# syncdoth/face_mask_inpaint

Measured on AMD Instinct MI355X. Metric: train images/sec at 256x256 bs=8 per GPU (PICNet-ref train step), higher is better.
Workload: dtype f32; 1 GPU; train_reference_fill.py PICNet-ref 256x256 fp32, bs=8 per GPU, synthetic CelebA-HQ-shaped batch + random binary_map (BASELINE configs[1]); global_batch=8, parallelism=dp1

## Files before the change

face_mask_inpaint_amd/_lib.py:

```python
from __future__ import annotations

import ctypes as C
import os

_HERE = os.path.dirname(os.path.abspath(__file__))
LIB_PATH = os.path.join(_HERE, "csrc", "libfmi_hip.so")

c_f = C.c_void_p
i32, i64, f32, vp = C.c_int, C.c_int64, C.c_float, C.c_void_p


class ConvDesc(C.Structure):

    _fields_ = [(n, C.c_int) for n in ("N", "H", "W", "C", "OH", "OW", "K", "x_cstride", "y_cstride", "kh", "kw", "stride", "pad", "pad_mode", "dil")] + [("w3", C.c_void_p), ("x3", C.c_void_p), ("y3", C.c_void_p)]


class WeightEntry(C.Structure):
    _fields_ = [("w", vp), ("u", vp), ("v", vp), ("wf", vp), ("wt", vp), ("sigma", vp), ("rows", i32), ("C", i32), ("taps", i32), ("iters", i32), ("wf3", vp), ("wt3", vp)]


class WeightGradEntry(C.Structure):
    _fields_ = [("w", vp), ("u", vp), ("v", vp), ("sigma", vp), ("dwf", vp), ("dw", vp), ("rows", i32), ("C", i32), ("taps", i32), ("pad_", i32)]


# ... 10 lines not shown
SIGNATURES = {
    "fmi_gemm_f32": [vp, vp, vp, i32, i32, i32, i64, i64, i64, i64, i64, i64, i32, i64, i64, i64, f32, f32, vp, vp],
    "fmi_ssim_valid_f32": [vp, vp, vp, i32, i32, i32, i32, f32, f32, vp, vp, i64, vp],
    "fmi_avgpool2_pad_f32": [vp, vp, i32, i32, i32, i32, i32, vp],
    "fmi_resample_u8": [vp, vp, i32, i32, i32, i32, i32, i32, i32, i32, vp, vp, i32, vp],
    "fmi_gather_u8_i64": [vp, vp, i32, i32, i32, i32, i32, vp, vp, vp],
    "fmi_u8_lut_chw_f32": [vp, vp, vp, i32, i32, i32, i32, vp],
    "fmi_split3_f32": [vp, vp, vp, i64, i32, i32, f32, vp],
    "fmi_split3_colsum_f32": [vp, vp, vp, i64, i32, vp],
    "fmi_merge3_f32": [vp, vp, i64, i32, vp],
    "fmi_conv2d_fwd_f32": [PD, vp, vp, vp, vp, vp, i32, i32, i64, vp],
    "fmi_conv2d_dgrad_f32": [PD, vp, vp, vp, vp, vp, i32, i64, vp],
    "fmi_conv_transpose2d_pair_f32": [PD, vp, vp, i32, vp, vp, vp, vp],
    "fmi_conv2d_dgrad_masked_f32": [PD, vp, vp, vp, f32, vp, vp],
    "fmi_conv2d_dgrad_masked_add_f32": [PD, vp, vp, vp, f32, vp, vp, vp],
    "fmi_conv2d_wgrad_f32": [PD, vp, vp, vp, vp, i32, i64, vp],
    "fmi_conv2d_thin_fwd_f32": [PD, vp, vp, vp, vp, vp, i32, vp],
    "fmi_conv2d_thin_dgrad_f32": [PD, vp, vp, vp, vp],
    "fmi_conv2d_thin_input_dgrad_f32": [PD, vp, vp, vp, vp],
    "fmi_conv2d_thin_lrelu_fwd_f32": [PD, vp, f32, vp, vp, vp, i32, vp],
    "fmi_conv2d_thin_lrelu_dgrad_f32": [PD, vp, vp, vp, f32, vp, vp],
    "fmi_conv2d_thin_lrelu_wgrad_f32": [PD, vp, f32, vp, vp, vp, vp],
    "fmi_conv2d_thin_wgrad_f32": [PD, vp, vp, vp, vp, vp],
    "fmi_conv2d_fwd_bf16": [PD, vp, vp, vp, vp, vp, i64, vp],
    "fmi_conv2d_dgrad_bf16": [PD, vp, vp, vp, vp, vp, i64, vp],
    "fmi_conv2d_wgrad_bf16": [PD, vp, vp, vp, vp],
    "fmi_pack_weight_bf16": [vp, vp, i32, i32, i32, vp],
    "fmi_scale_channels_bf16": [vp, vp, vp, i32, i64, i32, vp],
    "fmi_scale_channels_gs_bf16": [vp, vp, vp, vp, i64, i32, i64, i32, vp],
    "fmi_noise_bias_act_bf16": [vp, vp, vp, vp, vp, i64, i32, f32, f32, vp],
    "fmi_noise_bias_act_bwd_bf16": [vp, vp, vp, vp, vp, vp, vp, i64, i64, i32, f32, f32, vp],
    "fmi_upfirdn2d_nhwc_bf16": [vp, vp, vp] + [i32] * 14 + [vp],
    "fmi_styled_out_bwd_bf16": [vp] * 11 + [i64, vp, i32, i64, i32, f32, f32, vp],
    "fmi_conv2d_fwd_act_bf16": [PD, vp, vp, vp, vp, vp, vp, f32, f32, vp, vp],
    "fmi_blur_act_bf16": [vp, vp, vp] + [i32] * 8 + [vp, vp, vp, vp, f32, f32, i32, vp],
    "fmi_torgb_fwd_bf16": [vp, vp, vp, vp, vp, vp, i32, i64, i32, vp],
    "fmi_torgb_bwd_bf16": [vp, vp, vp, vp, vp, vp, i64, vp, vp, vp, i32, i64, i32, vp],
    "fmi_bias_grad_f32": [vp, i64, i32, i32, vp, vp],
    "fmi_reflect_pad_fold_f32": [vp, vp, i32, i32, i32, i32, i32, vp],
    "fmi_weight_prepare_f32": [vp, i32, vp],
    "fmi_weight_grad_f32": [vp, i32, vp, vp],
    "fmi_softmax_rows_f32": [vp, vp, i64, i32, vp],
    "fmi_softmax_rows_bwd_f32": [vp, vp, vp, i64, i32, vp],
    "fmi_attention_fwd_f32": [vp, vp, vp, vp, vp, vp, i32, i32, i32, i32, i32, vp],
    "fmi_attention_bwd_f32": [vp] * 12 + [i32] * 5 + [vp],
    "fmi_eltwise_f32": [i32, vp, vp, vp, i64, f32, vp],
# ... 56 lines not shown
    "fmi_adam_step_dev_guarded_f32": [vp, i32, f32, f32, f32, f32, f32, vp, vp, vp],
    "fmi_ranger_step_f32": [vp, i32, f32, f32, f32, f32, f32, f32, i32, f32, i32, vp],
    "fmi_upfirdn2d_f32": [vp, vp, vp, i32, i32, i32, i32, i32, i32, i32, i32, i32, i32, i32, i32, i32, vp],
    "fmi_upfirdn2d_bf16": [vp, vp, vp, i32, i32, i32, i32, i32, i32, i32, i32, i32, i32, i32, i32, i32, vp],
    "fmi_fused_bias_act_f32": [vp, vp, vp, vp, i64, i32, i32, i32, i32, f32, f32, vp],
    "fmi_fused_bias_act_bf16": [vp, vp, vp, vp, i64, i32, i32, i32, i32, f32, f32, vp],
    "fmi_scale_channels_f32": [vp, vp, vp, i32, i64, i32, vp],
    "fmi_scale_channels_gs_f32": [vp, vp, vp, vp, i64, i32, i64, i32, vp],
    "fmi_sqsum_last_f32": [vp, vp, i64, i32, vp],
    "fmi_sqsum_last_bwd_f32": [vp, vp, vp, i64, i32, vp],
    "fmi_noise_bias_act_bwd_f32": [vp, vp, vp, vp, vp, i64, i32, f32, f32, vp],
    "fmi_upfirdn2d_nhwc_f32": [vp, vp, vp, i32, i32, i32, i32, i32, i32, i32, i32, i32, i32, i32, i32, i32, i32, vp],
    "fmi_prelu_f32": [vp, vp, vp, i64, i32, vp],
    "fmi_prelu_bwd_f32": [vp, vp, vp, vp, vp, vp, i64, i64, i32, vp],
    "fmi_subsample_f32": [vp, vp, i32, i32, i32, i32, i32, i32, vp],
    "fmi_bias_grad_nchw_f32": [vp, i32, i32, i64, vp, vp],
    "fmi_bias_grad_nchw_bf16": [vp, i32, i32, i64, vp, vp],
    "fmi_noise_bias_act_f32": [vp, vp, vp, vp, vp, i64, i32, f32, f32, vp],
}

STATUS = {0: "ok", 1: "bad argument", 2: "unsupported shape/mode", 3: "kernel launch failed"}


PREDICATES = {"fmi_debug_bf16_tile": [i32], "fmi_set_deterministic": [i32], "fmi_get_deterministic": [], "fmi_conv2d_thin_supported": [PD], "fmi_conv2d_bf16_supported": [PD], "fmi_conv2d_thin_lrelu_supported": [PD]}


class FmiError(RuntimeError):
    pass


class Library:

    def __init__(self, path: str = LIB_PATH, strict: bool = True):
        if not os.path.exists(path):
            raise FmiError(
                f"{path} not found: build the HIP extension first (python -c 'import __graft_entry__ as g; g.build()'). "
                "There is no CPU fallback."
            )
        self.path = path
        self.cdll = C.CDLL(path)
        self.missing = []
        for name, argtypes in SIGNATURES.items():
            try:
                fn = getattr(self.cdll, name)
            except AttributeError:
                self.missing.append(name)
                continue
# ... 35 lines not shown
```

face_mask_inpaint_amd/csrc/thinconv.hip:

```cpp
#include "common.h"
#include <cstdlib>

namespace {

__device__ __forceinline__ int reflect1(int i, int n) {
  if (i < 0) i = -i;
  if (i >= n) i = 2 * n - 2 - i;
  return i;
}

struct ThinArgs {
  const float* x;
  const float* w;
  const float* bias;
  const float* res;
  float* y;
  int N, H, W, C, K, xcs, ycs, pad_mode, act;
  int flip = 0;
  float in_slope = 1.f;
  const float* xin = nullptr;
};
__device__ __forceinline__ float4 lrelu4(float4 v, float s) {
  v.x = v.x > 0.f ? v.x : v.x * s, v.y = v.y > 0.f ? v.y : v.y * s, v.z = v.z > 0.f ? v.z : v.z * s, v.w = v.w > 0.f ? v.w : v.w * s;
  return v;
// ... 247 lines not shown
      }
      for (int m = 4; m < 4 * CQ; m <<= 1)
#pragma unroll
        for (int k = 0; k < K; ++k) acc[k] += __shfl_xor(acc[k], m, 64);
      if (live && q == 0) {
        const int o = x * a.ycs;
#pragma unroll
        for (int k = 0; k < K; ++k) {
          float r = acc[k];
          if (a.bias) r += a.bias[k];
          if (rrow) r += rrow[o + k];
          if (a.act == 1) r = tanhf(r);
          else if (a.act == 2) r = fmaxf(r, 0.f);
          yrow[o + k] = r;
        }
      }
    }
  }
}


constexpr int LT_H = 8, LT_W = 32, LT_PITCH = 36;
template <int K>
__global__ void __launch_bounds__(256) thin_fwd_lds_kernel(ThinArgs a, int tiles_x, int tiles_y) {
  __shared__ __attribute__((aligned(16))) float sx[(LT_H + 2) * (LT_W + 2) * LT_PITCH];
  const int tid = threadIdx.x, lane = tid & 63, wid = tid >> 6;
  const int i = lane & 3, q = (lane >> 2) & 7, g = lane >> 5;
  int b = blockIdx.x;
  const int tx = b % tiles_x;
  b /= tiles_x;
  const int ty = b % tiles_y, n = b / tiles_y;
  const int y0 = ty * LT_H, x0 = tx * LT_W;
  float wr[9][4];
#pragma unroll
  for (int t = 0; t < 9; ++t)
#pragma unroll
    for (int e = 0; e < 4; ++e) wr[t][e] = i < K ? a.w[((int64_t)(a.flip ? 8 - t : t) * a.C + 4 * q + e) * K + i] : 0.f;
  const float* img = a.x + (int64_t)n * a.H * a.W * a.xcs;
  constexpr int NPIX = (LT_H + 2) * (LT_W + 2), NLD = (NPIX + 31) / 32;
  float4 stage[NLD];
#pragma unroll
  for (int j = 0; j < NLD; ++j) {
    const int p = (tid >> 3) + 32 * j;
    const int wy = p / (LT_W + 2), wx = p - wy * (LT_W + 2);
    int iy = y0 + wy - 1, ix = x0 + wx - 1;
    if (a.pad_mode) {
      iy = reflect1(iy, a.H);
      ix = reflect1(ix, a.W);
    }
    const bool ok = p < NPIX && (unsigned)iy < (unsigned)a.H && (unsigned)ix < (unsigned)a.W;
    stage[j] = make_float4(0.f, 0.f, 0.f, 0.f);
    if (ok) stage[j] = *reinterpret_cast<const float4*>(img + ((int64_t)iy * a.W + ix) * a.xcs + 4 * (tid & 7));
  }
  if (a.in_slope != 1.f) {
#pragma unroll
    for (int j = 0; j < NLD; ++j) stage[j] = lrelu4(stage[j], a.in_slope);
  }
#pragma unroll
  for (int j = 0; j < NLD; ++j) {
    const int p = (tid >> 3) + 32 * j;
    if (p < NPIX) *reinterpret_cast<float4*>(sx + p * LT_PITCH + 4 * (tid & 7)) = stage[j];
  }
  __syncthreads();
#pragma unroll 1
  for (int it = 0; it < 8; ++it) {
    const int ly = 2 * wid + (it >> 2), lx = (it & 3) * 8 + g * 4 + i;
    const float* base = sx + (ly * (LT_W + 2) + lx) * LT_PITCH + 4 * q;
    f32x4_t acc = {0.f, 0.f, 0.f, 0.f};
#pragma unroll
    for (int t = 0; t < 9; ++t) {
      const float4 v = *reinterpret_cast<const float4*>(base + ((t / 3) * (LT_W + 2) + (t % 3)) * LT_PITCH);
      acc = __builtin_amdgcn_mfma_f32_4x4x1f32(wr[t][0], v.x, acc, 0, 0, 0);
      acc = __builtin_amdgcn_mfma_f32_4x4x1f32(wr[t][1], v.y, acc, 0, 0, 0);
      acc = __builtin_amdgcn_mfma_f32_4x4x1f32(wr[t][2], v.z, acc, 0, 0, 0);
      acc = __builtin_amdgcn_mfma_f32_4x4x1f32(wr[t][3], v.w, acc, 0, 0, 0);
    }
#pragma unroll
    for (int m = 4; m < 32; m <<= 1)
#pragma unroll
      for (int k = 0; k < K; ++k) acc[k] += __shfl_xor(acc[k], m, 64);
    const int oy = y0 + ly, ox = x0 + lx;
    if (q < K && oy < a.H && ox < a.W) {
      const int64_t o = ((int64_t)(n * a.H + oy) * a.W + ox) * a.ycs + q;
      float r = acc[0];
#pragma unroll
      for (int k = 1; k < K; ++k) r = q == k ? acc[k] : r;
      if (a.bias) r += a.bias[q];
      if (a.res) r += a.res[o];
      if (a.act == 1) r = tanhf(r);
      else if (a.act == 2) r = fmaxf(r, 0.f);
      a.y[o] = r;
    }
  }
}


template <int K>
__global__ void __launch_bounds__(256) thin_wgrad_lds_kernel(ThinArgs a, float* __restrict__ dwf, float* __restrict__ dbias, int tiles_x,
                                                             int tiles_y, int ntiles) {
  __shared__ __attribute__((aligned(16))) float sx[(LT_H + 2) * (LT_W + 2) * LT_PITCH];
  float(*red)[8] = reinterpret_cast<float(*)[8]>(sx);
  const int tid = threadIdx.x, lane = tid & 63, wid = tid >> 6;
  const int j = lane & 7, grp = lane >> 3;
  float acc[9][4][K], bacc[K];
#pragma unroll
  for (int t = 0; t < 9; ++t)
#pragma unroll
    for (int e = 0; e < 4; ++e)
#pragma unroll
      for (int k = 0; k < K; ++k) acc[t][e][k] = 0.f;
#pragma unroll
  for (int k = 0; k < K; ++k) bacc[k] = 0.f;
  constexpr int NPIX = (LT_H + 2) * (LT_W + 2), NLD = (NPIX + 31) / 32;
  for (int tile = blockIdx.x; tile < ntiles; tile += gridDim.x) {
    int b = tile;
// ... 123 lines not shown
        if (!cok) px = 0;
#pragma unroll
        for (int r = 0; r < 3; ++r) {
          struct __attribute__((packed, aligned(4))) GK {
            float e[K];
          };
          const GK g = *reinterpret_cast<const GK*>(gp[r] + px * a.ycs);
#pragma unroll
          for (int k = 0; k < K; ++k) gv[r * 3 + c][k] = (cok && rok[r]) ? g.e[k] : 0.f;
        }
      }
      f32x4_t acc = {0.f, 0.f, 0.f, 0.f};
#pragma unroll
      for (int t = 0; t < 9; ++t)
#pragma unroll
        for (int k = 0; k < K; ++k) acc = __builtin_amdgcn_mfma_f32_4x4x1f32(wr[t][k], gv[t][k], acc, 0, 0, 0);
      if (live) {
        float4 o = make_float4(acc[0], acc[1], acc[2], acc[3]);
        if (a.xin) o = lrelu_mask4(o, *reinterpret_cast<const float4*>(a.xin + (xrow - dx) + (int64_t)x * a.xcs), a.in_slope);
        *reinterpret_cast<float4*>(xrow + (int64_t)x * a.xcs) = o;
      }
    }
  }
}

bool thin_shape_ok(const fmi_conv_desc* d) {
  const int cg = d->C / 4;
  return d->dil <= 1 && (int64_t)d->N * d->H * d->W < (1ll << 31) && d->K >= 1 && d->K <= 4 && d->kh == 3 && d->kw == 3 && d->stride == 1 && d->pad == 1 && d->C % 4 == 0 && cg >= 1 &&
         cg <= 16 && (cg & (cg - 1)) == 0 && d->x_cstride % 4 == 0 && d->H >= 3 && d->W >= 3 && d->OH == d->H && d->OW == d->W;
}

}

#define THIN_DISPATCH(KERNEL, ...)                                                              \
  switch (d->K) {                                                                               \
    case 1: hipLaunchKernelGGL((KERNEL<1>), dim3(grid), dim3(256), 0, st, __VA_ARGS__); break;  \
    case 2: hipLaunchKernelGGL((KERNEL<2>), dim3(grid), dim3(256), 0, st, __VA_ARGS__); break;  \
    case 3: hipLaunchKernelGGL((KERNEL<3>), dim3(grid), dim3(256), 0, st, __VA_ARGS__); break;  \
    default: hipLaunchKernelGGL((KERNEL<4>), dim3(grid), dim3(256), 0, st, __VA_ARGS__); break; \
  }

extern "C" int fmi_conv2d_thin_supported(const fmi_conv_desc* d) { return d && thin_shape_ok(d) ? 1 : 0; }

static bool thin_lrelu_ok(const fmi_conv_desc* d) { return thin_shape_ok(d) && d->C == 32; }
extern "C" int fmi_conv2d_thin_lrelu_supported(const fmi_conv_desc* d) { return d && thin_lrelu_ok(d) ? 1 : 0; }

static int thin_fwd_impl(const fmi_conv_desc* d, const float* x, float in_slope, const float* wf, const float* bias, const float* residual,
                         float* y, int act, void* stream) {
  if (!d || !x || !wf || !y || act < 0 || act > 2) return FMI_ERR_BAD_ARG;
  if (!thin_shape_ok(d) || ((uintptr_t)x & 15)) return FMI_ERR_UNSUPPORTED;
  if (in_slope != 1.f && !thin_lrelu_ok(d)) return FMI_ERR_UNSUPPORTED;
  hipStream_t st = (hipStream_t)stream;
  ThinArgs a{x, wf, bias, residual, y, d->N, d->H, d->W, d->C, d->K, d->x_cstride, d->y_cstride, d->pad_mode, act};
  a.in_slope = in_slope;
  const int G = d->C / 4;
  const int64_t total = (int64_t)d->N * d->H * d->W;
  if (total >= (1ll << 31)) return FMI_ERR_UNSUPPORTED;
  int qbits = 0;
  while ((1 << qbits) < G) ++qbits;
  if (d->C == 32) {
    const int tiles_x = (d->W + LT_W - 1) / LT_W, tiles_y = (d->H + LT_H - 1) / LT_H;
    const int64_t nb = (int64_t)d->N * tiles_x * tiles_y;
    if (nb < (1ll << 31)) {
      const int grid = (int)nb;
      THIN_DISPATCH(thin_fwd_lds_kernel, a, tiles_x, tiles_y);
      return fmi_launch_status();
    }
  }
  const int segs = (d->W + SEG - 1) / SEG, ntasks = d->N * d->H * segs;
  const int grid = ntasks / 4 > 8192 ? 8192 : (ntasks + 3) / 4;
  THIN_DISPATCH(thin_fwd_mfma_kernel, a, qbits, ntasks, segs);
  return fmi_launch_status();
}

extern "C" int fmi_conv2d_thin_fwd_f32(const fmi_conv_desc* d, const float* x, const float* wf, const float* bias,
                                       const float* residual, float* y, int act, void* stream) {
  return thin_fwd_impl(d, x, 1.f, wf, bias, residual, y, act, stream);
}
extern "C" int fmi_conv2d_thin_lrelu_fwd_f32(const fmi_conv_desc* d, const float* x, float in_slope, const float* wf, const float* bias,
                                             float* y, int act, void* stream) {
  return thin_fwd_impl(d, x, in_slope, wf, bias, nullptr, y, act, stream);
}

static int thin_dgrad_impl(const fmi_conv_desc* d, const float* dy, const float* wt, const float* xin, float in_slope, float* dx,
                           void* stream) {
  if (!d || !dy || !wt || !dx) return FMI_ERR_BAD_ARG;
  if (!thin_shape_ok(d) || ((uintptr_t)dx & 15) || ((uintptr_t)xin & 15)) return FMI_ERR_UNSUPPORTED;
  hipStream_t st = (hipStream_t)stream;
// ... 39 lines not shown
  const int grid = ntasks / 4 > 8192 ? 8192 : (ntasks + 3) / 4;
  switch (d->C) {
    case 1: hipLaunchKernelGGL((thin_fwd_mfma_kernel<1>), dim3(grid), dim3(256), 0, st, a, qbits, ntasks, segs); break;
    case 2: hipLaunchKernelGGL((thin_fwd_mfma_kernel<2>), dim3(grid), dim3(256), 0, st, a, qbits, ntasks, segs); break;
    case 3: hipLaunchKernelGGL((thin_fwd_mfma_kernel<3>), dim3(grid), dim3(256), 0, st, a, qbits, ntasks, segs); break;
    default: hipLaunchKernelGGL((thin_fwd_mfma_kernel<4>), dim3(grid), dim3(256), 0, st, a, qbits, ntasks, segs); break;
  }
  return fmi_launch_status();
}

static int thin_wgrad_impl(const fmi_conv_desc* d, const float* x, float in_slope, const float* dy, float* dwf, float* dbias, void* stream) {
  if (!d || !x || !dy || !dwf) return FMI_ERR_BAD_ARG;
  if (!thin_shape_ok(d) || ((uintptr_t)x & 15)) return FMI_ERR_UNSUPPORTED;
  if (in_slope != 1.f && !thin_lrelu_ok(d)) return FMI_ERR_UNSUPPORTED;
  hipStream_t st = (hipStream_t)stream;
  ThinArgs a{x, nullptr, nullptr, nullptr, const_cast<float*>(dy), d->N, d->H, d->W, d->C, d->K, d->x_cstride, d->y_cstride, d->pad_mode, 0};
  a.in_slope = in_slope;
  const int G = d->C / 4;
  const int64_t total = (int64_t)d->N * d->H * d->W;
  if (d->C == 32) {
    const int tiles_x = (d->W + LT_W - 1) / LT_W, tiles_y = (d->H + LT_H - 1) / LT_H;
    const int64_t nt = (int64_t)d->N * tiles_x * tiles_y;
    if (nt < (1ll << 31)) {
      const int grid = fmi_det() ? 1 : (nt < 768 ? (int)nt : 768);
      THIN_DISPATCH(thin_wgrad_lds_kernel, a, dwf, dbias, tiles_x, tiles_y, (int)nt);
      return fmi_launch_status();
    }
  }
  const int64_t waves = (total + 64 / G - 1) / (64 / G);
  const int grid = fmi_det() ? 1 : (int)(waves / 4 > 1024 ? 1024 : (waves + 3) / 4);
  THIN_DISPATCH(thin_wgrad_kernel, a, dwf, dbias, G, total);
  return fmi_launch_status();
}
extern "C" int fmi_conv2d_thin_wgrad_f32(const fmi_conv_desc* d, const float* x, const float* dy, float* dwf, float* dbias,
                                         void* stream) {
  return thin_wgrad_impl(d, x, 1.f, dy, dwf, dbias, stream);
}
extern "C" int fmi_conv2d_thin_lrelu_wgrad_f32(const fmi_conv_desc* d, const float* x, float in_slope, const float* dy, float* dwf,
                                               float* dbias, void* stream) {
  return thin_wgrad_impl(d, x, in_slope, dy, dwf, dbias, stream);
}
```

face_mask_inpaint_amd/functional.py:

```python
from __future__ import annotations

import ctypes as C
import math
from typing import List, Optional, Sequence, Tuple

import torch

from . import _lib
from ._lib import ConvDesc, FmiError

EW_LRELU, EW_LRELU_BWD, EW_TANH_BWD, EW_ADD, EW_SCALE, EW_AXPY, EW_MUL, EW_RELU_BWD_OUT, EW_SOFTPLUS, EW_SOFTPLUS_BWD, EW_SUB, EW_RSQRT, EW_RSQRT_BWD, EW_SIGMOID, EW_SIGMOID_BWD = range(15)
ACT_NONE, ACT_TANH, ACT_RELU = 0, 1, 2

ATTN_CHUNK_BYTES = 96 * 1024 * 1024

PROFILE = None


class _prof:
    def __init__(self, tag, flops):
        self.tag, self.flops = tag, flops

    def __enter__(self):
        if PROFILE is not None:
# ... 369 lines not shown


class _ThinConvLReLU(torch.autograd.Function):

    @staticmethod
    def forward(ctx, x, wf, bias, wt, slope, pad_mode, act):
        _chk(x, wf, bias)
        n, h, w, c = x.shape
        k = wf.shape[2]
        d, oh, ow = conv_desc(n, h, w, c, k, 3, 3, 1, 1, pad_mode)
        y = torch.empty((n, oh, ow, k), device=x.device, dtype=torch.float32)
        with _prof(f"conv_fwd|{n}x{h}x{w} {c}->{k} k3s1", 2.0 * n * oh * ow * k * c * 9):
            _L().conv2d_thin_lrelu_fwd_f32(C.byref(d), _p(x), slope, _p(wf), _p(bias), _p(y), act, _st())
        ctx.save_for_backward(x, wf, y if act else None)
        ctx.wt, ctx.cfg, ctx.has_b = wt, (slope, pad_mode, act), bias is not None
        return y

    @staticmethod
    def backward(ctx, gy):
        lib = _L()
        x, wf, y = ctx.saved_tensors
        slope, pad_mode, act = ctx.cfg
        gy = gy.contiguous()
        if act:
            gy = _act_bwd(gy, y, act)
        n, h, w, c = x.shape
        k = wf.shape[2]
        d, _, _ = conv_desc(n, h, w, c, k, 3, 3, 1, 1, pad_mode)
        gx = gwf = gb = None
        if ctx.needs_input_grad[0]:
            gx = torch.empty_like(x)
            with _prof(f"conv_dgrad|{n}x{h}x{w} {c}->{k} k3s1", 2.0 * gy.numel() * c * 9):
                lib.conv2d_thin_lrelu_dgrad_f32(C.byref(d), _p(gy), _p(ctx.wt), _p(x), slope, _p(gx), _st())
        if ctx.needs_input_grad[1]:
            gwf = _zeros_like(wf)
            if ctx.has_b and ctx.needs_input_grad[2]:
                gb = _zeros(k, x.device, torch.float32)
            with _prof(f"conv_wgrad|{n}x{h}x{w} {c}->{k} k3s1", 2.0 * gy.numel() * c * 9):
                lib.conv2d_thin_lrelu_wgrad_f32(C.byref(d), _p(x), slope, _p(gy), _p(gwf), _p(gb), _st())
        elif ctx.has_b and ctx.needs_input_grad[2]:
            gb = _zeros(k, x.device, torch.float32)
            lib.bias_grad_f32(_p(gy), gy.numel() // k, k, k, _p(gb), _st())
        return gx, gwf, gb, None, None, None, None


def lrelu_conv2d(x, pw: PackedWeight, bias=None, slope=0.1, pad=1, pad_mode=0, act=ACT_NONE):
    if x.dtype == torch.float32 and pw.kh == 3 and pw.kw == 3 and pad == 1 and x.is_cuda:
        n, h, w, c = x.shape
        d, _, _ = conv_desc(n, h, w, c, pw.wf.shape[2], 3, 3, 1, 1, pad_mode)
        if _L().conv2d_thin_lrelu_supported(C.byref(d)) and x.data_ptr() % 16 == 0:
            return _ThinConvLReLU.apply(x, pw.wf, bias, pw.wt, float(slope), pad_mode, act)
    return conv2d(leaky_relu(x, slope), pw, bias, None, 1, pad, pad_mode, act)
# ... 1718 lines not shown
```

include/fmi_hip.h:

```cpp
#ifndef FMI_HIP_H
#define FMI_HIP_H

#include <stdint.h>

#ifdef __cplusplus
extern "C" {
#endif

typedef enum {
  FMI_OK = 0,
  FMI_ERR_BAD_ARG = 1,
  FMI_ERR_UNSUPPORTED = 2,
  FMI_ERR_LAUNCH = 3
} fmi_status;

const char* fmi_status_string(int status);
int fmi_version(void);
int fmi_set_deterministic(int on);
int fmi_get_deterministic(void);

int fmi_debug_bf16_tile(int mode);

int fmi_gemm_f32(const float* A, const float* B, float* C, int M, int N, int K,
                 int64_t sa_m, int64_t sa_k, int64_t sb_k, int64_t sb_n, int64_t sc_m, int64_t sc_n,
// ... 27 lines not shown
                       const float* residual, float* y, int act, int batch_w, int64_t w_bstride, void* stream);
int fmi_conv_transpose2d_pair_f32(const fmi_conv_desc* d, const float* x1, const float* x2, int K2, const void* w3b, const float* bias,
                                  float* y, void* stream);
int fmi_conv2d_dgrad_f32(const fmi_conv_desc* d, const float* dy, const float* wt, const float* bias,
                         const float* residual, float* dx, int batch_w, int64_t w_bstride, void* stream);
int fmi_conv2d_dgrad_masked_f32(const fmi_conv_desc* d, const float* dy, const float* wt, const float* mask, float mask_slope, float* dx,
                                void* stream);
int fmi_conv2d_dgrad_masked_add_f32(const fmi_conv_desc* d, const float* dy, const float* wt, const float* mask, float mask_slope,
                                    const float* gadd, float* dx, void* stream);
int fmi_conv2d_wgrad_f32(const fmi_conv_desc* d, const float* x, const float* dy, float* dwf, float* dbias,
                         int batch_w, int64_t w_bstride, void* stream);
int fmi_conv2d_thin_supported(const fmi_conv_desc* d);
int fmi_conv2d_thin_fwd_f32(const fmi_conv_desc* d, const float* x, const float* wf, const float* bias,
                            const float* residual, float* y, int act, void* stream);
int fmi_conv2d_thin_dgrad_f32(const fmi_conv_desc* d, const float* dy, const float* wt, float* dx, void* stream);
int fmi_conv2d_thin_wgrad_f32(const fmi_conv_desc* d, const float* x, const float* dy, float* dwf, float* dbias, void* stream);
int fmi_conv2d_thin_lrelu_supported(const fmi_conv_desc* d);
int fmi_conv2d_thin_lrelu_fwd_f32(const fmi_conv_desc* d, const float* x, float in_slope, const float* wf, const float* bias, float* y, int act,
                                  void* stream);
int fmi_conv2d_thin_lrelu_dgrad_f32(const fmi_conv_desc* d, const float* dy, const float* wt, const float* x, float in_slope, float* dx,
                                    void* stream);
int fmi_conv2d_thin_lrelu_wgrad_f32(const fmi_conv_desc* d, const float* x, float in_slope, const float* dy, float* dwf, float* dbias,
                                    void* stream);
int fmi_conv2d_thin_input_dgrad_f32(const fmi_conv_desc* d, const float* dy, const float* wt, float* dx, void* stream);
int fmi_conv2d_bf16_supported(const fmi_conv_desc* d);
int fmi_conv2d_fwd_bf16(const fmi_conv_desc* d, const uint16_t* x, const uint16_t* wnk, const float* colscale, uint16_t* y, float* ws,
                        int64_t ws_floats, void* stream);
int fmi_conv2d_fwd_act_bf16(const fmi_conv_desc* d, const uint16_t* x, const uint16_t* wnk, const float* colscale, const float* noise,
                            const float* nw, const float* bias, float slope, float gain, uint16_t* y, void* stream);
int fmi_conv2d_dgrad_bf16(const fmi_conv_desc* d, const uint16_t* dy, const uint16_t* wck, const float* colscale, uint16_t* dx, float* ws,
                          int64_t ws_floats, void* stream);
int fmi_conv2d_wgrad_bf16(const fmi_conv_desc* d, const uint16_t* x, const uint16_t* dy, float* dwf, void* stream);
int fmi_pack_weight_bf16(const float* src_tab, uint16_t* dst_bta, int T, int A, int B, void* stream);
int fmi_scale_channels_bf16(const uint16_t* x, const float* s, uint16_t* y, int N, int64_t P, int C, void* stream);
int fmi_scale_channels_gs_bf16(const uint16_t* g, const uint16_t* x, float* gs, float* ws, int64_t ws_floats, int N, int64_t P, int C,
                               void* stream);
int fmi_noise_bias_act_bf16(const uint16_t* x, const float* bias, const float* noise, const float* nw, uint16_t* y, int64_t pixels, int C,
                            float alpha, float scale, void* stream);
int fmi_noise_bias_act_bwd_bf16(const uint16_t* g, const uint16_t* y, const float* noise, uint16_t* gx, float* gnw, float* gbias,
                                float* ws, int64_t ws_floats, int64_t pixels, int C, float alpha, float scale, void* stream);
int fmi_upfirdn2d_nhwc_bf16(const uint16_t* in, const float* kernel, uint16_t* out, int N, int in_h, int in_w, int C, int kh, int kw,
                            int up_x, int up_y, int down_x, int down_y, int pad_x0, int pad_x1, int pad_y0, int pad_y1, void* stream);
int fmi_blur_act_bf16(const uint16_t* in, const float* kernel, uint16_t* out, int N, int in_h, int in_w, int C, int pad_x0, int pad_x1,
                      int pad_y0, int pad_y1, const float* colscale, const float* noise, const float* nw, const float* bias, float slope,
                      float gain, int separable, void* stream);
int fmi_styled_out_bwd_bf16(const uint16_t* g, const uint16_t* y, const float* noise, const float* colscale, const float* nw,
// ... 206 lines not shown
```

Baseline: 102.3 images/s.

## Fuse thin lrelu conv dgrad, wgrad and tanh backward into one persistent kernel

Adds a fused backward kernel for the thin (few output channel) 3x3 conv with input leaky-relu. In one pass it computes the input gradient, the weight and bias gradients via per-block partial rows and a row-sum reduction, and optionally applies the tanh derivative, with reflect-pad folding handled separately for border tiles. The forward LDS kernel becomes persistent with prefetch of the next tile window, and the wgrad grid is sized from occupancy queries. This aims to cut separate dgrad/wgrad/activation launches and repeated reads of x and dy, at the cost of a workspace allocation and considerable kernel complexity.

```diff
diff --git a/face_mask_inpaint_amd/_lib.py b/face_mask_inpaint_amd/_lib.py
--- a/face_mask_inpaint_amd/_lib.py
+++ b/face_mask_inpaint_amd/_lib.py
@@ -56,6 +56,7 @@
     "fmi_conv2d_thin_lrelu_dgrad_f32": [PD, vp, vp, vp, f32, vp, vp],
     "fmi_conv2d_thin_lrelu_wgrad_f32": [PD, vp, f32, vp, vp, vp, vp],
     "fmi_conv2d_thin_wgrad_f32": [PD, vp, vp, vp, vp, vp],
+    "fmi_conv2d_thin_lrelu_bwd_f32": [PD, vp, f32, vp, vp, vp, vp, vp, vp, vp, i64, vp],
     "fmi_conv2d_fwd_bf16": [PD, vp, vp, vp, vp, vp, i64, vp],
     "fmi_conv2d_dgrad_bf16": [PD, vp, vp, vp, vp, vp, i64, vp],
     "fmi_conv2d_wgrad_bf16": [PD, vp, vp, vp, vp],
@@ -158,7 +159,7 @@
 STATUS = {0: "ok", 1: "bad argument", 2: "unsupported shape/mode", 3: "kernel launch failed"}
 
 
-PREDICATES = {"fmi_debug_bf16_tile": [i32], "fmi_set_deterministic": [i32], "fmi_get_deterministic": [], "fmi_conv2d_thin_supported": [PD], "fmi_conv2d_bf16_supported": [PD], "fmi_conv2d_thin_lrelu_supported": [PD]}
+PREDICATES = {"fmi_debug_bf16_tile": [i32], "fmi_set_deterministic": [i32], "fmi_get_deterministic": [], "fmi_conv2d_thin_supported": [PD], "fmi_conv2d_bf16_supported": [PD], "fmi_conv2d_thin_lrelu_supported": [PD], "fmi_conv2d_thin_lrelu_bwd_ws_bytes": [PD]}
 
 
 class FmiError(RuntimeError):
diff --git a/face_mask_inpaint_amd/csrc/thinconv.hip b/face_mask_inpaint_amd/csrc/thinconv.hip
--- a/face_mask_inpaint_amd/csrc/thinconv.hip
+++ b/face_mask_inpaint_amd/csrc/thinconv.hip
@@ -293,75 +293,98 @@
 
 constexpr int LT_H = 8, LT_W = 32, LT_PITCH = 36;
 template <int K>
-__global__ void __launch_bounds__(256) thin_fwd_lds_kernel(ThinArgs a, int tiles_x, int tiles_y) {
+__global__ void __launch_bounds__(256) thin_fwd_lds_kernel(ThinArgs a, int tiles_x, int tiles_y, int ntiles) {
   __shared__ __attribute__((aligned(16))) float sx[(LT_H + 2) * (LT_W + 2) * LT_PITCH];
   const int tid = threadIdx.x, lane = tid & 63, wid = tid >> 6;
   const int i = lane & 3, q = (lane >> 2) & 7, g = lane >> 5;
-  int b = blockIdx.x;
-  const int tx = b % tiles_x;
-  b /= tiles_x;
-  const int ty = b % tiles_y, n = b / tiles_y;
-  const int y0 = ty * LT_H, x0 = tx * LT_W;
   float wr[9][4];
 #pragma unroll
   for (int t = 0; t < 9; ++t)
 #pragma unroll
     for (int e = 0; e < 4; ++e) wr[t][e] = i < K ? a.w[((int64_t)(a.flip ? 8 - t : t) * a.C + 4 * q + e) * K + i] : 0.f;
-  const float* img = a.x + (int64_t)n * a.H * a.W * a.xcs;
   constexpr int NPIX = (LT_H + 2) * (LT_W + 2), NLD = (NPIX + 31) / 32;
   float4 stage[NLD];
-#pragma unroll
-  for (int j = 0; j < NLD; ++j) {
-    const int p = (tid >> 3) + 32 * j;
-    const int wy = p / (LT_W + 2), wx = p - wy * (LT_W + 2);
-    int iy = y0 + wy - 1, ix = x0 + wx - 1;
-    if (a.pad_mode) {
-      iy = reflect1(iy, a.H);
-      ix = reflect1(ix, a.W);
-    }
-    const bool ok = p < NPIX && (unsigned)iy < (unsigned)a.H && (unsigned)ix < (unsigned)a.W;
-    stage[j] = make_float4(0.f, 0.f, 0.f, 0.f);
-    if (ok) stage[j] = *reinterpret_cast<const float4*>(img + ((int64_t)iy * a.W + ix) * a.xcs + 4 * (tid & 7));
-  }
-  if (a.in_slope != 1.f) {
-#pragma unroll
-    for (int j = 0; j < NLD; ++j) stage[j] = lrelu4(stage[j], a.in_slope);
-  }
-#pragma unroll
-  for (int j = 0; j < NLD; ++j) {
-    const int p = (tid >> 3) + 32 * j;
-    if (p < NPIX) *reinterpret_cast<float4*>(sx + p * LT_PITCH + 4 * (tid & 7)) = stage[j];
-  }
-  __syncthreads();
+  auto load_window = [&](int tile) {
+    const int tx = tile % tiles_x;
+    tile /= tiles_x;
+    const int ty = tile % tiles_y, n = tile / tiles_y;
+    const int y0 = ty * LT_H, x0 = tx * LT_W;
+    const float* img = a.x + (int64_t)n * a.H * a.W * a.xcs;
+#pragma unroll
+    for (int j = 0; j < NLD; ++j) {
+      const int p = (tid >> 3) + 32 * j;
+      const int wy = p / (LT_W + 2), wx = p - wy * (LT_W + 2);
+      int iy = y0 + wy - 1, ix = x0 + wx - 1;
+      if (a.pad_mode) {
+        iy = reflect1(iy, a.H);
+        ix = reflect1(ix, a.W);
+      }
+      const bool ok = p < NPIX && (unsigned)iy < (unsigned)a.H && (unsigned)ix < (unsigned)a.W;
+      stage[j] = make_float4(0.f, 0.f, 0.f, 0.f);
+      if (ok) stage[j] = *reinterpret_cast<const float4*>(img + ((int64_t)iy * a.W + ix) * a.xcs + 4 * (tid & 7));
+    }
+  };
+  int tile = blockIdx.x;
+  load_window(tile);
+  while (true) {
+    if (a.in_slope != 1.f) {
+#pragma unroll
+      for (int j = 0; j < NLD; ++j) stage[j] = lrelu4(stage[j], a.in_slope);
+    }
+#pragma unroll
+    for (int j = 0; j < NLD; ++j) {
+      const int p = (tid >> 3) + 32 * j;
+      if (p < NPIX) *reinterpret_cast<float4*>(sx + p * LT_PITCH + 4 * (tid & 7)) = stage[j];
+    }
+    __syncthreads();
+    int b = tile;
+    const int tx = b % tiles_x;
+    b /= tiles_x;
+    const int ty = b % tiles_y, n = b / tiles_y;
+    const int y0 = ty * LT_H, x0 = tx * LT_W;
+    const int next = tile + gridDim.x;
+    if (next < ntiles) load_window(next);
+    float fin[K];
+#pragma unroll
+    for (int k = 0; k < K; ++k) fin[k] = 0.f;
 #pragma unroll 1
-  for (int it = 0; it < 8; ++it) {
-    const int ly = 2 * wid + (it >> 2), lx = (it & 3) * 8 + g * 4 + i;
-    const float* base = sx + (ly * (LT_W + 2) + lx) * LT_PITCH + 4 * q;
-    f32x4_t acc = {0.f, 0.f, 0.f, 0.f};
-#pragma unroll
-    for (int t = 0; t < 9; ++t) {
-      const float4 v = *reinterpret_cast<const float4*>(base + ((t / 3) * (LT_W + 2) + (t % 3)) * LT_PITCH);
-      acc = __builtin_amdgcn_mfma_f32_4x4x1f32(wr[t][0], v.x, acc, 0, 0, 0);
-      acc = __builtin_amdgcn_mfma_f32_4x4x1f32(wr[t][1], v.y, acc, 0, 0, 0);
-      acc = __builtin_amdgcn_mfma_f32_4x4x1f32(wr[t][2], v.z, acc, 0, 0, 0);
-      acc = __builtin_amdgcn_mfma_f32_4x4x1f32(wr[t][3], v.w, acc, 0, 0, 0);
-    }
-#pragma unroll
-    for (int m = 4; m < 32; m <<= 1)
-#pragma unroll
-      for (int k = 0; k < K; ++k) acc[k] += __shfl_xor(acc[k], m, 64);
-    const int oy = y0 + ly, ox = x0 + lx;
-    if (q < K && oy < a.H && ox < a.W) {
-      const int64_t o = ((int64_t)(n * a.H + oy) * a.W + ox) * a.ycs + q;
-      float r = acc[0];
-#pragma unroll
-      for (int k = 1; k < K; ++k) r = q == k ? acc[k] : r;
-      if (a.bias) r += a.bias[q];
-      if (a.res) r += a.res[o];
-      if (a.act == 1) r = tanhf(r);
-      else if (a.act == 2) r = fmaxf(r, 0.f);
-      a.y[o] = r;
-    }
+    for (int it = 0; it < 8; ++it) {
+      const int ly = 2 * wid + (it >> 2), lx = (it & 3) * 8 + g * 4 + i;
+      const float* base = sx + (ly * (LT_W + 2) + lx) * LT_PITCH + 4 * q;
+      f32x4_t acc = {0.f, 0.f, 0.f, 0.f};
+#pragma unroll
+      for (int t = 0; t < 9; ++t) {
+        const float4 v = *reinterpret_cast<const float4*>(base + ((t / 3) * (LT_W + 2) + (t % 3)) * LT_PITCH);
+        acc = __builtin_amdgcn_mfma_f32_4x4x1f32(wr[t][0], v.x, acc, 0, 0, 0);
+        acc = __builtin_amdgcn_mfma_f32_4x4x1f32(wr[t][1], v.y, acc, 0, 0, 0);
+        acc = __builtin_amdgcn_mfma_f32_4x4x1f32(wr[t][2], v.z, acc, 0, 0, 0);
+        acc = __builtin_amdgcn_mfma_f32_4x4x1f32(wr[t][3], v.w, acc, 0, 0, 0);
+      }
+#pragma unroll
+      for (int m = 4; m < 32; m <<= 1)
+#pragma unroll
+        for (int k = 0; k < K; ++k) acc[k] += __shfl_xor(acc[k], m, 64);
+#pragma unroll
+      for (int k = 0; k < K; ++k) fin[k] = it == q ? acc[k] : fin[k];
+    }
+    {
+      const int oy = y0 + 2 * wid + (q >> 2), ox = x0 + (q & 3) * 8 + g * 4 + i;
+      if (oy < a.H && ox < a.W) {
+        const int64_t o = ((int64_t)(n * a.H + oy) * a.W + ox) * a.ycs;
+#pragma unroll
+        for (int k = 0; k < K; ++k) {
+          float r = fin[k];
+          if (a.bias) r += a.bias[k];
+          if (a.res) r += a.res[o + k];
+          if (a.act == 1) r = tanhf(r);
+          else if (a.act == 2) r = fmaxf(r, 0.f);
+          a.y[o + k] = r;
+        }
+      }
+    }
+    if (next >= ntiles) break;
+    tile = next;
+    __syncthreads();
   }
 }
 
@@ -531,6 +554,339 @@
       }
     }
   }
+}
+
+constexpr int BW_W = LT_W + 2, BW_CELLS = (LT_H + 2) * (LT_W + 2), BW_LD = (BW_CELLS + 255) / 256;
+constexpr int BWD_MAX_ROWS = 2048;
+
+template <int P>
+__device__ __forceinline__ float quad_bcast(float v) {
+  return __builtin_bit_cast(float, __builtin_amdgcn_update_dpp(0, __builtin_bit_cast(int, v), P * 0x55, 0xf, 0xf, true));
+}
+
+struct FoldFlags {
+  bool y0, y2, x0, x2;
+};
+__device__ __forceinline__ FoldFlags fold_flags(int pad_mode, int oy, int ox, int H, int W) {
+  FoldFlags f;
+  f.y0 = pad_mode && oy == 1, f.y2 = pad_mode && oy == H - 2, f.x0 = pad_mode && ox == 1, f.x2 = pad_mode && ox == W - 2;
+  return f;
+}
+__device__ __forceinline__ float4 sel4(bool c, float4 v) { return c ? v : make_float4(0.f, 0.f, 0.f, 0.f); }
+__device__ __forceinline__ float4 add4(float4 a, float4 b) { return make_float4(a.x + b.x, a.y + b.y, a.z + b.z, a.w + b.w); }
+
+template <bool FOLD, int TY, int TX>
+__device__ __forceinline__ float4 bwd_g4(const float4* wp, FoldFlags f) {
+  constexpr int o = (2 - TY) * BW_W + (2 - TX);
+  constexpr int dr = (TY == 0 ? -2 : 2) * BW_W, dc = TX == 0 ? -2 : 2;
+  float4 v = wp[o];
+  if constexpr (FOLD) {
+    const bool ey = TY == 0 ? f.y0 : TY == 2 ? f.y2 : false, ex = TX == 0 ? f.x0 : TX == 2 ? f.x2 : false;
+    if constexpr (TY != 1) v = add4(v, sel4(ey, wp[o + dr]));
+    if constexpr (TX != 1) v = add4(v, sel4(ex, wp[o + dc]));
+    if constexpr (TY != 1 && TX != 1) v = add4(v, sel4(ey && ex, wp[o + dr + dc]));
+  }
+  return v;
+}
+template <bool FOLD, int TY, int TX>
+__device__ __forceinline__ float bwd_g1(const float* w1, FoldFlags f) {
+  constexpr int o = 4 * ((2 - TY) * BW_W + (2 - TX));
+  constexpr int dr = 4 * (TY == 0 ? -2 : 2) * BW_W, dc = 4 * (TX == 0 ? -2 : 2);
+  float v = w1[o];
+  if constexpr (FOLD) {
+    const bool ey = TY == 0 ? f.y0 : TY == 2 ? f.y2 : false, ex = TX == 0 ? f.x0 : TX == 2 ? f.x2 : false;
+    if constexpr (TY != 1) v += ey ? w1[o + dr] : 0.f;
+    if constexpr (TX != 1) v += ex ? w1[o + dc] : 0.f;
+    if constexpr (TY != 1 && TX != 1) v += (ey && ex) ? w1[o + dr + dc] : 0.f;
+  }
+  return v;
+}
+
+struct BwdTile {
+  int n, y0, x0;
+};
+struct BwdTiling {
+  int tiles_x, tiles_y, ix0, ix1, iy0, iy1;
+  __host__ __device__ int iw() const { return ix1 - ix0; }
+  __host__ __device__ int ih() const { return iy1 - iy0; }
+  __host__ __device__ int per_image(bool border) const { return border ? tiles_x * tiles_y - iw() * ih() : iw() * ih(); }
+};
+template <bool BORDER>
+__device__ __forceinline__ BwdTile bwd_tile(int tile, const BwdTiling& g) {
+  BwdTile t;
+  const int per = g.per_image(BORDER);
+  t.n = tile / per;
+  int j = tile - t.n * per, tx, ty;
+  if (!BORDER) {
+    ty = g.iy0 + j / g.iw();
+    tx = g.ix0 + j % g.iw();
+  } else {
+    const int full = (g.tiles_y - g.ih()) * g.tiles_x;
+    if (j < full) {
+      const int r = j / g.tiles_x;
+      tx = j - r * g.tiles_x;
+      ty = r < g.iy0 ? r : r - g.iy0 + g.iy1;
+    } else {
+      j -= full;
+      const int side = g.tiles_x - g.iw(), r = j / side, c = j - r * side;
+      ty = g.iy0 + r;
+      tx = c < g.ix0 ? c : c - g.ix0 + g.ix1;
+    }
+  }
+  t.y0 = ty * LT_H, t.x0 = tx * LT_W;
+  return t;
+}
+
+struct BwdArgs {
+  const float* x;
+  const float* dy;
+  const float* yt;
+  const float* wt;
+  float* dx;
+  float* ws;
+  int N, H, W, xcs, ycs, pad_mode;
+  float slope;
+};
+
+template <int K>
+struct __attribute__((packed, aligned(4))) GKv {
+  float e[K];
+};
+
+template <int K>
+__device__ __forceinline__ void bwd_win_load(const BwdArgs& a, BwdTile t, int tid, GKv<K> (&g)[BW_LD], GKv<K> (&yv)[BW_LD], bool (&inner)[BW_LD]) {
+#pragma unroll
+  for (int l = 0; l < BW_LD; ++l) {
+    const int p = tid + 256 * l;
+    const int wy = p / BW_W, wx = p - wy * BW_W;
+    const int py = t.y0 + wy - 1, px = t.x0 + wx - 1;
+    const bool ok = p < BW_CELLS && (unsigned)py < (unsigned)a.H && (unsigned)px < (unsigned)a.W;
+    inner[l] = ok && wy >= 1 && wy <= LT_H && wx >= 1 && wx <= LT_W;
+#pragma unroll
+    for (int k = 0; k < K; ++k) g[l].e[k] = 0.f, yv[l].e[k] = 0.f;
+    if (ok) {
+      const int64_t o = ((int64_t)(t.n * a.H + py) * a.W + px) * a.ycs;
+      g[l] = *reinterpret_cast<const GKv<K>*>(a.dy + o);
+      if (a.yt) yv[l] = *reinterpret_cast<const GKv<K>*>(a.yt + o);
+    }
+  }
+}
+template <int K>
+__device__ __forceinline__ void bwd_win_store(float4* win, int tid, const GKv<K> (&g)[BW_LD], const GKv<K> (&yv)[BW_LD], const bool (&inner)[BW_LD],
+                                              float (&bacc)[K]) {
+#pragma unroll
+  for (int l = 0; l < BW_LD; ++l) {
+    const int p = tid + 256 * l;
+    float v[4] = {0.f, 0.f, 0.f, 0.f};
+#pragma unroll
+    for (int k = 0; k < K; ++k) {
+      v[k] = g[l].e[k] * (1.f - yv[l].e[k] * yv[l].e[k]);
+      bacc[k] += inner[l] ? v[k] : 0.f;
+    }
+    if (p < BW_CELLS) win[p] = make_float4(v[0], v[1], v[2], v[3]);
+  }
+}
+
+__device__ __forceinline__ int64_t bwd_x_uoff(const BwdArgs& a, BwdTile t, int it) {
+  return ((int64_t)(t.n * a.H + t.y0 + (it >> 2)) * a.W + t.x0 + (it & 3) * 8) * a.xcs;
+}
+struct BwdLane {
+  int xlo;
+  int ry, rx;
+};
+__device__ __forceinline__ float4 bwd_x_load(const BwdArgs& a, BwdTile t, int it, BwdLane l, bool valid) {
+  const bool in = valid && t.y0 + l.ry + (it >> 2) < a.H && t.x0 + l.rx + (it & 3) * 8 < a.W;
+  const float* p = a.x + bwd_x_uoff(a, t, it) + l.xlo;
+  return *reinterpret_cast<const float4*>(in ? p : a.x);
+}
+
+constexpr int BWD_PF = 4;
+template <int K, bool FOLD>
+__device__ __forceinline__ void bwd_tile_compute(const BwdArgs& a, const float4* win, BwdTile t, BwdTile nx, bool hasn, BwdLane l, int g, int i,
+                                                 const float (&wr)[9][K], f32x4_t (&dw)[9], float4 (&xr)[BWD_PF]) {
+  static_assert(BWD_PF == 4, "one pass of the unrolled loop = one tile row of the wave");
+#pragma unroll
+  for (int h = 0; h < 2; ++h) {
+    const float4* wrow = win + (l.ry + h) * BW_W + l.rx;
+    const float* grow = reinterpret_cast<const float*>(win + (l.ry + h) * BW_W + 4 * g) + i;
+    const int oy = t.y0 + l.ry + h;
+#pragma unroll
+    for (int j = 0; j < 4; ++j) {
+      const int it = 4 * h + j;
+      const int ox = t.x0 + l.rx + 8 * j;
+      const bool live = oy < a.H && ox < a.W;
+      const float4 xv = sel4(live, xr[j]);
+      xr[j] = h == 0 ? bwd_x_load(a, t, it + 4, l, true) : bwd_x_load(a, nx, it - 4, l, hasn);
+      {
+        const FoldFlags f = fold_flags(a.pad_mode, oy, ox, a.H, a.W);
+        f32x4_t acc[3];
+#pragma unroll
+        for (int r = 0; r < 3; ++r) acc[r] = f32x4_t{0.f, 0.f, 0.f, 0.f};
+#define BWD_TAP(TY, TX)                                                                                                                  \
+  {                                                                                                                                      \
+    const float4 gq = bwd_g4<FOLD, TY, TX>(wrow + 8 * j, f);                                                                             \
+    const float ge[4] = {gq.x, gq.y, gq.z, gq.w};                                                                                        \
+    _Pragma("unroll") for (int k = 0; k < K; ++k) acc[TY] = __builtin_amdgcn_mfma_f32_4x4x1f32(wr[TY * 3 + TX][k], ge[k], acc[TY], 0, 0, 0); \
+  }
+        BWD_TAP(0, 0) BWD_TAP(1, 0) BWD_TAP(2, 0) BWD_TAP(0, 1) BWD_TAP(1, 1) BWD_TAP(2, 1) BWD_TAP(0, 2) BWD_TAP(1, 2) BWD_TAP(2, 2)
+#undef BWD_TAP
+        if (live) {
+          const float4 o = make_float4(acc[0][0] + acc[1][0] + acc[2][0], acc[0][1] + acc[1][1] + acc[2][1], acc[0][2] + acc[1][2] + acc[2][2],
+                                       acc[0][3] + acc[1][3] + acc[2][3]);
+          *reinterpret_cast<float4*>(a.dx + bwd_x_uoff(a, t, it) + l.xlo) = lrelu_mask4(o, xv, a.slope);
+        }
+      }
+      const float4 lv = lrelu4(xv, a.slope);
+#define BWD_PIX(P)                                                                                                                           \
+  {                                                                                                                                          \
+    const float b0 = quad_bcast<P>(lv.x), b1 = quad_bcast<P>(lv.y), b2 = quad_bcast<P>(lv.z), b3 = quad_bcast<P>(lv.w);                      \
+    const float b = i == 0 ? b0 : i == 1 ? b1 : i == 2 ? b2 : b3;                                             \
+    const FoldFlags f = fold_flags(a.pad_mode, oy, t.x0 + 4 * g + 8 * j + P, a.H, a.W);                                                      \
+    BWD_WTAP(P, 0, 0) BWD_WTAP(P, 0, 1) BWD_WTAP(P, 0, 2) BWD_WTAP(P, 1, 0) BWD_WTAP(P, 1, 1) BWD_WTAP(P, 1, 2) BWD_WTAP(P, 2, 0) BWD_WTAP(P, 2, 1) \
+    BWD_WTAP(P, 2, 2)                                                                                                                        \
+  }
+#define BWD_WTAP(P, TY, TX) dw[TY * 3 + TX] = __builtin_amdgcn_mfma_f32_4x4x1f32(bwd_g1<FOLD, TY, TX>(grow + 4 * (8 * j + P), f), b, dw[TY * 3 + TX], 0, 0, 0);
+      BWD_PIX(0) BWD_PIX(1) BWD_PIX(2) BWD_PIX(3)
+#undef BWD_WTAP
+#undef BWD_PIX
+    }
+  }
+}
+
+template <int K, bool FOLD>
+__global__ void __launch_bounds__(256) __attribute__((amdgpu_waves_per_eu((!FOLD && K <= 3) ? 3 : 2))) thin_lrelu_bwd_kernel(BwdArgs a, BwdTiling tg, int ntiles, int row0) {
+  __shared__ __attribute__((aligned(16))) float4 win[2][BW_CELLS];
+  __shared__ float red[9 * 4 * 32];
+  __shared__ float lds4[4];
+  const int tid = threadIdx.x, lane = tid & 63, wid = tid >> 6;
+  const int i = lane & 3, q = (lane >> 2) & 7, g = lane >> 5;
+  float wr[9][K];
+#pragma unroll
+  for (int t = 0; t < 9; ++t)
+#pragma unroll
+    for (int k = 0; k < K; ++k) wr[t][k] = a.wt[(t * K + k) * 32 + 4 * q + i];
+  f32x4_t dw[9];
+#pragma unroll
+  for (int t = 0; t < 9; ++t) dw[t] = f32x4_t{0.f, 0.f, 0.f, 0.f};
+  float bacc[K];
+#pragma unroll
+  for (int k = 0; k < K; ++k) bacc[k] = 0.f;
+  GKv<K> sg[BW_LD], sy[BW_LD];
+  bool inner[BW_LD];
+  float4 xr[BWD_PF];
+
+  int tile = blockIdx.x;
+  BwdTile cur = bwd_tile<FOLD>(tile, tg);
+  bwd_win_load<K>(a, cur, tid, sg, sy, inner);
+  const BwdLane l{(2 * wid * a.W + 4 * g + i) * a.xcs + 4 * q, 2 * wid, 4 * g + i};
+#pragma unroll
+  for (int it = 0; it < BWD_PF; ++it) xr[it] = bwd_x_load(a, cur, it, l, true);
+  bwd_win_store<K>(win[0], tid, sg, sy, inner, bacc);
+  __syncthreads();
+  int pb = 0;
+  for (; tile < ntiles; tile += gridDim.x) {
+    const bool hasn = tile + (int)gridDim.x < ntiles;
+    const BwdTile nx = bwd_tile<FOLD>(hasn ? tile + gridDim.x : tile, tg);
+    if (hasn) bwd_win_load<K>(a, nx, tid, sg, sy, inner);
+    bwd_tile_compute<K, FOLD>(a, win[pb], cur, nx, hasn, l, g, i, wr, dw, xr);
+    if (hasn) bwd_win_store<K>(win[pb ^ 1], tid, sg, sy, inner, bacc);
+    __syncthreads();
+    pb ^= 1;
+    cur = nx;
+  }
+#pragma unroll
+  for (int t = 0; t < 9; ++t)
+#pragma unroll
+    for (int r = 0; r < 4; ++r) dw[t][r] += __shfl_xor(dw[t][r], 32, 64);
+  for (int w = 0; w < 4; ++w) {
+    if (wid == w && g == 0) {
+#pragma unroll
+      for (int t = 0; t < 9; ++t)
+#pragma unroll
+        for (int r = 0; r < 4; ++r) {
+          float* p = red + (t * 4 + r) * 32 + (lane & 31);
+          *p = w == 0 ? dw[t][r] : *p + dw[t][r];
+        }
+    }
+    __syncthreads();
+  }
+  constexpr int RW = 9 * 32 * K + K;
+  float* row = a.ws + (int64_t)(row0 + blockIdx.x) * RW;
+  for (int idx = tid; idx < 9 * 32 * K; idx += 256) {
+    const int t = idx / (32 * K), rem = idx - t * 32 * K, c = rem / K, k = rem - c * K;
+    row[idx] = red[(t * 4 + k) * 32 + c];
+  }
+#pragma unroll
+  for (int k = 0; k < K; ++k) {
+    const float s_ = block_sum_256(bacc[k], lds4);
+    if (tid == 0) row[9 * 32 * K + k] = s_;
+  }
+}
+
+__global__ void __launch_bounds__(1024) thin_sum_rows_kernel(const float* __restrict__ ws, float* __restrict__ dwf, float* __restrict__ dbias, int rows,
+                                                             int width, int nw) {
+  __shared__ float part[32][33];
+  const int tx = threadIdx.x & 31, ty = threadIdx.x >> 5;
+  const int i = blockIdx.x * 32 + tx;
+  float s4[4] = {0.f, 0.f, 0.f, 0.f};
+  if (i < width) {
+    int r = ty;
+    for (; r + 96 < rows; r += 128) {
+#pragma unroll
+      for (int u = 0; u < 4; ++u) s4[u] += ws[(int64_t)(r + 32 * u) * width + i];
+    }
+    for (int u = 0; r < rows; r += 32, ++u) s4[u] += ws[(int64_t)r * width + i];
+  }
+  part[ty][tx] = (s4[0] + s4[1]) + (s4[2] + s4[3]);
+  __syncthreads();
+  if (ty == 0 && i < width) {
+    float t = 0.f;
+#pragma unroll
+    for (int l = 0; l < 32; ++l) t += part[l][tx];
+    if (i < nw) dwf[i] = t;
+    else if (dbias) dbias[i - nw] = t;
+  }
+}
+
+template <typename F>
+static int resident_grid(F kernel) {
+  int per_cu = 0, dev = 0, cus = 0;
+  if (hipOccupancyMaxActiveBlocksPerMultiprocessor(&per_cu, kernel, 256, 0) != hipSuccess || per_cu < 1) per_cu = 1;
+  if (hipGetDevice(&dev) != hipSuccess || hipDeviceGetAttribute(&cus, hipDeviceAttributeMultiprocessorCount, dev) != hipSuccess || cus < 1) cus = 256;
+  (void)hipGetLastError();
+  return per_cu * cus;
+}
+template <int K, bool FOLD>
+static int bwd_resident_grid() {
+  static const int g = resident_grid(thin_lrelu_bwd_kernel<K, FOLD>);
+  return g;
+}
+template <int K>
+static void bwd_launch(const fmi_conv_desc* d, const BwdArgs& a, int64_t rows, hipStream_t st, int* rows_used) {
+  BwdTiling tg{(d->W + LT_W - 1) / LT_W, (d->H + LT_H - 1) / LT_H, 0, 0, 0, 0};
+  if (!d->pad_mode) tg.ix1 = tg.tiles_x, tg.iy1 = tg.tiles_y;
+  else if ((d->H - 2) / LT_H > 1 && (d->W - 2) / LT_W > 1) tg.ix0 = 1, tg.ix1 = (d->W - 2) / LT_W, tg.iy0 = 1, tg.iy1 = (d->H - 2) / LT_H;
+  const int64_t n_in = (int64_t)d->N * tg.per_image(false), n_bd = (int64_t)d->N * tg.per_image(true);
+  int64_t g_in = bwd_resident_grid<K, false>(), g_bd = bwd_resident_grid<K, true>();
+  if (g_in > n_in) g_in = n_in;
+  if (g_bd > n_bd) g_bd = n_bd;
+  if (g_in + g_bd > rows) {
+    if (g_bd > rows / 4) g_bd = n_bd ? (rows / 4 > 1 ? rows / 4 : 1) : 0;
+    if (g_in > rows - g_bd) g_in = rows - g_bd;
+  }
+  if (g_in > 0) hipLaunchKernelGGL((thin_lrelu_bwd_kernel<K, false>), dim3((unsigned)g_in), dim3(256), 0, st, a, tg, (int)n_in, 0);
+  if (g_bd > 0) hipLaunchKernelGGL((thin_lrelu_bwd_kernel<K, true>), dim3((unsigned)g_bd), dim3(256), 0, st, a, tg, (int)n_bd, (int)g_in);
+  *rows_used = (int)(g_in + g_bd);
+}
+template <int K>
+static int fwd_lds_resident_grid() {
+  static const int g = resident_grid(thin_fwd_lds_kernel<K>);
+  return g;
+}
+template <int K>
+static int wgrad_lds_resident_grid() {
+  static const int g = resident_grid(thin_wgrad_lds_kernel<K>);
+  return g;
 }
 
 bool thin_shape_ok(const fmi_conv_desc* d) {
@@ -571,8 +927,15 @@
     const int tiles_x = (d->W + LT_W - 1) / LT_W, tiles_y = (d->H + LT_H - 1) / LT_H;
     const int64_t nb = (int64_t)d->N * tiles_x * tiles_y;
     if (nb < (1ll << 31)) {
-      const int grid = (int)nb;
-      THIN_DISPATCH(thin_fwd_lds_kernel, a, tiles_x, tiles_y);
+      int res = 768;
+      switch (d->K) {
+        case 1: res = fwd_lds_resident_grid<1>(); break;
+        case 2: res = fwd_lds_resident_grid<2>(); break;
+        case 3: res = fwd_lds_resident_grid<3>(); break;
+        default: res = fwd_lds_resident_grid<4>(); break;
+      }
+      const int grid = (int)(nb < res ? nb : res);
+      THIN_DISPATCH(thin_fwd_lds_kernel, a, tiles_x, tiles_y, (int)nb);
       return fmi_launch_status();
     }
   }
@@ -658,7 +1021,14 @@
     const int tiles_x = (d->W + LT_W - 1) / LT_W, tiles_y = (d->H + LT_H - 1) / LT_H;
     const int64_t nt = (int64_t)d->N * tiles_x * tiles_y;
     if (nt < (1ll << 31)) {
-      const int grid = fmi_det() ? 1 : (nt < 768 ? (int)nt : 768);
+      int res = 512;
+      switch (d->K) {
+        case 1: res = wgrad_lds_resident_grid<1>(); break;
+        case 2: res = wgrad_lds_resident_grid<2>(); break;
+        case 3: res = wgrad_lds_resident_grid<3>(); break;
+        default: res = wgrad_lds_resident_grid<4>(); break;
+      }
+      const int grid = fmi_det() ? 1 : (nt < res ? (int)nt : res);
       THIN_DISPATCH(thin_wgrad_lds_kernel, a, dwf, dbias, tiles_x, tiles_y, (int)nt);
       return fmi_launch_status();
     }
@@ -676,3 +1046,37 @@
                                                float* dbias, void* stream) {
   return thin_wgrad_impl(d, x, in_slope, dy, dwf, dbias, stream);
 }
+
+static int bwd_rows(const fmi_conv_desc* d) {
+  const int64_t nt = (int64_t)d->N * ((d->W + LT_W - 1) / LT_W) * ((d->H + LT_H - 1) / LT_H);
+  return (int)(nt < BWD_MAX_ROWS ? nt : BWD_MAX_ROWS);
+}
+extern "C" int fmi_conv2d_thin_lrelu_bwd_ws_bytes(const fmi_conv_desc* d) {
+  if (!d || !thin_lrelu_ok(d)) return 0;
+  return bwd_rows(d) * (9 * d->C * d->K + d->K) * (int)sizeof(float);
+}
+extern "C" int fmi_conv2d_thin_lrelu_bwd_f32(const fmi_conv_desc* d, const float* x, float in_slope, const float* dy, const float* y, const float* wt,
+                                             float* dx, float* dwf, float* dbias, void* ws, int64_t ws_bytes, void* stream) {
+  if (!d || !x || !dy || !wt || !dx || !dwf || !ws) return FMI_ERR_BAD_ARG;
+  if (!thin_lrelu_ok(d) || ((uintptr_t)x & 15) || ((uintptr_t)dx & 15) || ((uintptr_t)ws & 3)) return FMI_ERR_UNSUPPORTED;
+  const int tiles_x = (d->W + LT_W - 1) / LT_W, tiles_y = (d->H + LT_H - 1) / LT_H;
+  const int64_t nt = (int64_t)d->N * tiles_x * tiles_y;
+  if (nt >= (1ll << 31)) return FMI_ERR_UNSUPPORTED;
+  const int width = 9 * d->C * d->K + d->K;
+  int64_t rows = ws_bytes / ((int64_t)width * (int64_t)sizeof(float));
+  if (rows > bwd_rows(d)) rows = bwd_rows(d);
+  if (rows < 1) return FMI_ERR_BAD_ARG;
+  const bool two_sets = d->pad_mode && (d->H - 2) / LT_H > 1 && (d->W - 2) / LT_W > 1;
+  if (two_sets && rows < 2) return FMI_ERR_BAD_ARG;
+  hipStream_t st = (hipStream_t)stream;
+  BwdArgs a{x, dy, y, wt, dx, (float*)ws, d->N, d->H, d->W, d->x_cstride, d->y_cstride, d->pad_mode, in_slope};
+  int used = 0;
+  switch (d->K) {
+    case 1: bwd_launch<1>(d, a, rows, st, &used); break;
+    case 2: bwd_launch<2>(d, a, rows, st, &used); break;
+    case 3: bwd_launch<3>(d, a, rows, st, &used); break;
+    default: bwd_launch<4>(d, a, rows, st, &used); break;
+  }
+  hipLaunchKernelGGL(thin_sum_rows_kernel, dim3((width + 31) / 32), dim3(1024), 0, st, (const float*)ws, dwf, dbias, used, width, 9 * d->C * d->K);
+  return fmi_launch_status();
+}
diff --git a/face_mask_inpaint_amd/functional.py b/face_mask_inpaint_amd/functional.py
--- a/face_mask_inpaint_amd/functional.py
+++ b/face_mask_inpaint_amd/functional.py
@@ -415,12 +415,27 @@
         x, wf, y = ctx.saved_tensors
         slope, pad_mode, act = ctx.cfg
         gy = gy.contiguous()
-        if act:
-            gy = _act_bwd(gy, y, act)
         n, h, w, c = x.shape
         k = wf.shape[2]
         d, _, _ = conv_desc(n, h, w, c, k, 3, 3, 1, 1, pad_mode)
         gx = gwf = gb = None
+        if ctx.needs_input_grad[0] and ctx.needs_input_grad[1]:
+            yt = None
+            if act == ACT_TANH:
+                yt = y
+            elif act:
+                gy = _act_bwd(gy, y, act)
+            gx = torch.empty_like(x)
+            gwf = torch.empty(wf.shape, device=x.device, dtype=torch.float32)
+            if ctx.has_b and ctx.needs_input_grad[2]:
+                gb = torch.empty(k, device=x.device, dtype=torch.float32)
+            ws_bytes = lib.conv2d_thin_lrelu_bwd_ws_bytes(C.byref(d))
+            ws = torch.empty(ws_bytes // 4, device=x.device, dtype=torch.float32)
+            with _prof(f"conv_bwd|{n}x{h}x{w} {c}->{k} k3s1", 4.0 * gy.numel() * c * 9):
+                lib.conv2d_thin_lrelu_bwd_f32(C.byref(d), _p(x), slope, _p(gy), _p(yt), _p(ctx.wt), _p(gx), _p(gwf), _p(gb), _p(ws), ws_bytes, _st())
+            return gx, gwf, gb, None, None, None, None
+        if act:
+            gy = _act_bwd(gy, y, act)
         if ctx.needs_input_grad[0]:
             gx = torch.empty_like(x)
             with _prof(f"conv_dgrad|{n}x{h}x{w} {c}->{k} k3s1", 2.0 * gy.numel() * c * 9):
diff --git a/include/fmi_hip.h b/include/fmi_hip.h
--- a/include/fmi_hip.h
+++ b/include/fmi_hip.h
@@ -73,6 +73,9 @@
                                     void* stream);
 int fmi_conv2d_thin_lrelu_wgrad_f32(const fmi_conv_desc* d, const float* x, float in_slope, const float* dy, float* dwf, float* dbias,
                                     void* stream);
+int fmi_conv2d_thin_lrelu_bwd_ws_bytes(const fmi_conv_desc* d);
+int fmi_conv2d_thin_lrelu_bwd_f32(const fmi_conv_desc* d, const float* x, float in_slope, const float* dy, const float* y, const float* wt,
+                                  float* dx, float* dwf, float* dbias, void* ws, int64_t ws_bytes, void* stream);
 int fmi_conv2d_thin_input_dgrad_f32(const fmi_conv_desc* d, const float* dy, const float* wt, float* dx, void* stream);
 int fmi_conv2d_bf16_supported(const fmi_conv_desc* d);
 int fmi_conv2d_fwd_bf16(const fmi_conv_desc* d, const uint16_t* x, const uint16_t* wnk, const float* colscale, uint16_t* y, float* ws,
```

Result: faster. 103.5 images/s (median of 6 runs) (+1.2%).
